# fmfi-compbio/nadavca

Hardware: AMD Instinct MI355X
Metric: reads/sec (align_signal, ~4k-sample reads) (higher is better)
Workload: dtype f64

## Files before the change

include/nadavca_hip.h:

```cpp
#ifndef NADAVCA_HIP_H
#define NADAVCA_HIP_H

#include <stddef.h>
#include <stdint.h>

#ifdef __cplusplus
extern "C" {
#endif

typedef struct nvk_ctx nvk_ctx;
typedef struct nvk_model nvk_model;

enum {
  NVK_OK = 0,
  NVK_ERR_NO_DEVICE = -1,
  NVK_ERR_INVALID = -2,
  NVK_ERR_HIP = -3,
  NVK_ERR_UNSUPPORTED = -4,
  NVK_ERR_NOMEM = -5
};

enum {
  NVK_READ_OK = 0,
  NVK_READ_NO_PATH = 1,
// ... 25 lines not shown
int nvk_ctx_synchronize(nvk_ctx *ctx);
void *nvk_ctx_stream(nvk_ctx *ctx);
int nvk_ctx_set_slots(nvk_ctx *ctx, int slots);

int nvk_timing_enable(nvk_ctx *ctx, int on);
int nvk_timing_reset(nvk_ctx *ctx);
int nvk_timing_read(nvk_ctx *ctx, int kernel_id, double *total_ms, int64_t *launches);
int nvk_last_batch_stats(nvk_ctx *ctx, int64_t *band_cells, int64_t *wave_steps,
                         int64_t *spill_bytes);
int nvk_last_retry_count(nvk_ctx *ctx, int64_t *n_reads);
enum { NVK_TIE_EXACT = 1, NVK_TIE_NEAR = 2, NVK_TIE_ULP = 4, NVK_TIE_PLATEAU = 8 };
int nvk_last_tie_count(nvk_ctx *ctx, int64_t *n_reads);
int nvk_last_tie_counts(nvk_ctx *ctx, int64_t *n_exact, int64_t *n_near, int64_t *n_ulp);
int nvk_last_tie_flags(nvk_ctx *ctx, int64_t n_reads, int32_t *out_flags);
int nvk_ctx_set_workspace_limit(nvk_ctx *ctx, int64_t bytes);

int nvk_model_create(nvk_ctx *ctx, int k, int central_position, int alphabet_size,
                     const double *mean, const double *sigma, int64_t n, nvk_model **out);
void nvk_model_destroy(nvk_model *model);
int nvk_model_info(const nvk_model *model, int *k, int *central_position, int *alphabet_size);

int nvk_expected_signal_batch(nvk_model *model, int64_t n_reads, const int32_t *reference,
                              const int64_t *ref_off, const int32_t *ctx_before,
                              const int64_t *cb_off, const int32_t *ctx_after,
                              const int64_t *ca_off, double *out);
int nvk_expected_signal_batch_dev(nvk_model *model, int64_t n_reads, int64_t total_ref,
                                  const int32_t *reference, const int64_t *ref_off,
                                  const int32_t *ctx_before, const int64_t *cb_off,
                                  const int32_t *ctx_after, const int64_t *ca_off, double *out);

// ... 104 lines not shown
```

nadavca_amd/_lib.py:

```python
import ctypes as C
import os
import threading

_HERE = os.path.dirname(os.path.abspath(__file__))
LIB_PATH = os.path.join(_HERE, 'csrc', 'libnadavca_hip.so')

NVK_OK = 0
NVK_ERR_NO_DEVICE = -1
NVK_ERR_INVALID = -2
NVK_ERR_HIP = -3
NVK_ERR_UNSUPPORTED = -4
NVK_ERR_NOMEM = -5

READ_OK = 0
READ_NO_PATH = 1
READ_BAD_INPUT = -1
READ_BAD_BAND = -2
READ_TOO_WIDE = -3

TIE_EXACT = 1
TIE_NEAR = 2
TIE_PLATEAU = 8
TIE_ULP = 4

# ... 12 lines not shown
    'nvk_device_count': (_int, []),
    'nvk_ctx_create': (_int, [_int, C.POINTER(_vp)]),
    'nvk_ctx_destroy': (None, [_vp]),
    'nvk_ctx_synchronize': (_int, [_vp]),
    'nvk_ctx_stream': (_vp, [_vp]),
    'nvk_ctx_set_slots': (_int, [_vp, _int]),
    'nvk_timing_enable': (_int, [_vp, _int]),
    'nvk_timing_reset': (_int, [_vp]),
    'nvk_timing_read': (_int, [_vp, _int, C.POINTER(_dbl), C.POINTER(_i64)]),
    'nvk_last_batch_stats': (_int, [_vp, C.POINTER(_i64), C.POINTER(_i64), C.POINTER(_i64)]),
    'nvk_last_retry_count': (_int, [_vp, C.POINTER(_i64)]),
    'nvk_last_tie_count': (_int, [_vp, C.POINTER(_i64)]),
    'nvk_last_tie_counts': (_int, [_vp, C.POINTER(_i64), C.POINTER(_i64), C.POINTER(_i64)]),
    'nvk_last_tie_flags': (_int, [_vp, _i64, _vp]),
    'nvk_ctx_set_workspace_limit': (_int, [_vp, _i64]),
    'nvk_model_create': (_int, [_vp, _int, _int, _int, _vp, _vp, _i64, C.POINTER(_vp)]),
    'nvk_model_destroy': (None, [_vp]),
    'nvk_model_info': (_int, [_vp, C.POINTER(_int), C.POINTER(_int), C.POINTER(_int)]),
    'nvk_expected_signal_batch': (_int, [_vp, _i64] + [_vp] * 7),
    'nvk_expected_signal_batch_dev': (_int, [_vp, _i64, _i64] + [_vp] * 7),
    'nvk_refine_alignment_batch': (_int, [_vp, _i64] + [_vp] * 10 + [_int, _int, _int, _vp, _vp]),
    'nvk_refine_alignment_submit': (_int, [_vp, _i64] + [_vp] * 10 + [_int, _int, _int, _vp, _vp, _vp, C.POINTER(_i64)]),
    'nvk_refine_alignment_wait': (_int, [_vp, _i64]),
    'nvk_refine_alignment_batch_dev': (_int, [_vp, _i64, _i64, _i64, _i64] + [_vp] * 10 + [_int, _int, _int, _vp, _vp]),
    'nvk_estimate_log_likelihoods_batch': (_int, [_vp, _i64] + [_vp] * 10 + [_int, _int, _int, _vp, _vp]),
    'nvk_estimate_log_likelihoods_batch_dev': (_int, [_vp, _i64, _i64, _i64, _i64] + [_vp] * 10 + [_int, _int, _int, _vp, _vp]),
    'nvk_consensus_accumulate_dev': (_int, [_vp, _i64, _i64, _int] + [_vp] * 6 + [_dbl, _i64, _vp, _vp]),
    'nvk_posterior_segments_dev': (_int, [_vp, _i64, _i64, _vp, _int, _int, _dbl, _vp, _vp, _vp]),
    'nvk_normalize_groups_dev': (_int, [_vp, _i64, _vp, _vp, _vp, _vp]),
    'nvk_select_hist_dev': (_int, [_vp, _vp, _i64, _int, _dbl, C.c_uint64, _int, _vp]),
# ... 93 lines not shown
        check(self._lib.nvk_last_retry_count(self.handle, C.byref(d)), 'nvk_last_retry_count')
        e = _i64()
        check(self._lib.nvk_last_tie_count(self.handle, C.byref(e)), 'nvk_last_tie_count')
        f, g, h = _i64(), _i64(), _i64()
        check(self._lib.nvk_last_tie_counts(self.handle, C.byref(f), C.byref(g), C.byref(h)), 'nvk_last_tie_counts')
        return dict(band_cells=a.value, wave_steps=b.value, spill_bytes=c.value, reads_redone_exact=d.value,
                    reads_tie_ambiguous=e.value, reads_tie_exact=f.value, reads_tie_near=g.value,
                    reads_tie_ulp=h.value)

    def last_tie_flags(self, n_reads):
        import numpy as np
        out = np.zeros(int(n_reads), dtype=np.int32)
        check(self._lib.nvk_last_tie_flags(self.handle, int(n_reads), _vp(out.ctypes.data)), 'nvk_last_tie_flags')
        return out

    def set_workspace_limit(self, nbytes):
        check(self._lib.nvk_ctx_set_workspace_limit(self.handle, int(nbytes)), 'nvk_ctx_set_workspace_limit')

    def close(self):
        if getattr(self, 'handle', None):
            self._lib.nvk_ctx_destroy(self.handle)
            self.handle = None

    def __del__(self):
        try:
            self.close()
        except Exception:
            pass


# ... 14 lines not shown
```

nadavca_amd/csrc/api.hip:

```cpp
#include <math.h>
#include <stdarg.h>
#include <stdio.h>
#include <stdlib.h>
#include <string.h>

#include <new>
#include <vector>

#include "nvk_internal.h"

static thread_local char g_err[512] = "";

void nvk_set_error(const char *fmt, ...) {
  va_list ap;
  va_start(ap, fmt);
  vsnprintf(g_err, sizeof g_err, fmt, ap);
  va_end(ap);
}

extern "C" const char *nvk_last_error(void) { return g_err; }

extern "C" int nvk_device_count(void) {
  int n = 0;
  if (hipGetDeviceCount(&n) != hipSuccess) return 0;
// ... 71 lines not shown
    nvk_set_error("no HIP device visible (this library has no CPU fallback)");
    return NVK_ERR_NO_DEVICE;
  }
  if (device < 0 || device >= n) {
    nvk_set_error("device %d out of range (0..%d)", device, n - 1);
    return NVK_ERR_INVALID;
  }
  NVK_HIP(hipSetDevice(device));
  nvk_ctx *c = new (std::nothrow) nvk_ctx();
  if (!c) {
    nvk_set_error("nvk_ctx_create: out of host memory");
    return NVK_ERR_NOMEM;
  }
  memset(c, 0, sizeof *c);
  c->device = device;
  hipDeviceProp_t prop;
  if (hipGetDeviceProperties(&prop, device) != hipSuccess) {
    delete c;
    nvk_set_error("hipGetDeviceProperties failed");
    return NVK_ERR_HIP;
  }
  c->num_cus = prop.multiProcessorCount > 0 ? prop.multiProcessorCount : 256;
  if (hipStreamCreate(&c->stream) != hipSuccess || hipStreamCreate(&c->stream2) != hipSuccess ||
      hipEventCreate(&c->ev0) != hipSuccess || hipEventCreate(&c->ev1) != hipSuccess ||
      hipEventCreateWithFlags(&c->ev_fork, hipEventDisableTiming) != hipSuccess ||
      hipEventCreateWithFlags(&c->ev_join, hipEventDisableTiming) != hipSuccess) {
    nvk_ctx_destroy(c);
    nvk_set_error("stream/event creation failed");
    return NVK_ERR_HIP;
  }
// ... 72 lines not shown

extern "C" int nvk_last_tie_count(nvk_ctx *ctx, int64_t *n_reads) {
  if (!ctx || !n_reads) return NVK_ERR_INVALID;
  *n_reads = ctx->last_ties;
  return NVK_OK;
}

extern "C" int nvk_last_tie_counts(nvk_ctx *ctx, int64_t *n_exact, int64_t *n_near, int64_t *n_ulp) {
  if (!ctx) return NVK_ERR_INVALID;
  if (n_exact) *n_exact = ctx->last_ties_exact;
  if (n_near) *n_near = ctx->last_ties_near;
  if (n_ulp) *n_ulp = ctx->last_ties_ulp;
  return NVK_OK;
}

extern "C" int nvk_last_tie_flags(nvk_ctx *ctx, int64_t n_reads, int32_t *out_flags) {
  if (!ctx || !out_flags || n_reads < 0) return NVK_ERR_INVALID;
  if (n_reads != ctx->ties_n) {
    nvk_set_error("nvk_last_tie_flags: the last refine_alignment batch had %lld reads, not %lld",
                  (long long)ctx->ties_n, (long long)n_reads);
    return NVK_ERR_INVALID;
  }
  if (n_reads == 0) return NVK_OK;
  if (ctx->ties_host) {
    memcpy(out_flags, ctx->ties_host, (size_t)n_reads * sizeof(int32_t));
    return NVK_OK;
  }
  NVK_HIP(hipSetDevice(ctx->device));
  NVK_HIP(hipMemcpyAsync(out_flags, ctx->ws[WS_TIES], (size_t)n_reads * sizeof(int32_t), hipMemcpyDeviceToHost,
                         ctx->stream));
// ... 155 lines not shown
}

struct PlanHost {
  PlanTotals tot;
  int32_t steps[1];
};

int plan_batch(nvk_model *model, const BatchArgs &a, int mode, int wobbling, PlanTotals &tot, const int **order,
               const int32_t **steps_sorted) {
  nvk_ctx *ctx = model->ctx;
  int64_t n = a.n_reads;
  int64_t rows_total = (mode == PLAN_ALIGN_TRANS) ? 2 * a.total_ref : a.total_ref + n;
  int rc;
  if ((rc = nvk_ws_reserve(ctx, WS_META, (size_t)(n + 1) * sizeof(ReadMeta) + 64))) return rc;
  if ((rc = nvk_ws_reserve(ctx, WS_ROWS, (size_t)(rows_total + 1) * sizeof(RowParam)))) return rc;
  if ((rc = nvk_ws_reserve(ctx, WS_BANDTMP, (size_t)(2 * (a.total_ref + n) + 2) * 8))) return rc;
  if ((rc = nvk_ws_reserve(ctx, WS_MISC, 256))) return rc;
  if ((rc = nvk_ws_reserve(ctx, WS_LANE_F, (size_t)(rows_total + 1) * 48))) return rc;
  if ((rc = nvk_ws_reserve(ctx, WS_LANE_R, (size_t)(rows_total + 1) * 48))) return rc;
  if ((rc = nvk_ws_reserve(ctx, WS_OFFS, (size_t)(rows_total + 1) * sizeof(int32_t)))) return rc;
  if ((rc = nvk_ws_reserve(ctx, WS_STEPS, (size_t)(n + 1) * sizeof(int32_t)))) return rc;
  if ((rc = nvk_grow(&ctx->h_plan, &ctx->h_plan_cap, sizeof(PlanHost) + (size_t)n * sizeof(int32_t), true,
                     "planner results")))
    return rc;
  PlanHost *hp = (PlanHost *)ctx->h_plan;
  PlanTotals *d_tot = (PlanTotals *)((char *)ctx->ws[WS_MISC] + 64);
  rc = launch_plan(ctx, model->dm, a, mode, wobbling, (ReadMeta *)ctx->ws[WS_META],
                   (RowParam *)ctx->ws[WS_ROWS], (unsigned long long *)ctx->ws[WS_BANDTMP], d_tot,
                   ctx->ws[WS_LANE_F], ctx->ws[WS_LANE_R], (int32_t *)ctx->ws[WS_OFFS]);
  if (rc) return rc;
  int *ord = nullptr;
  rc = launch_order(ctx, (const ReadMeta *)ctx->ws[WS_META], n, d_tot, &ord, (int32_t *)ctx->ws[WS_STEPS]);
  if (rc) return rc;
  NVK_HIP(hipMemcpyAsync(&hp->tot, d_tot, sizeof(PlanTotals), hipMemcpyDeviceToHost, ctx->stream));
  if (n) NVK_HIP(hipMemcpyAsync(hp->steps, ctx->ws[WS_STEPS], (size_t)n * sizeof(int32_t), hipMemcpyDeviceToHost,
                                ctx->stream));
  NVK_HIP(hipStreamSynchronize(ctx->stream));
  tot = hp->tot;
  *order = ord;
  *steps_sorted = hp->steps;
  ctx->last_cells = (int64_t)tot.cells;
  ctx->last_steps = (int64_t)tot.steps;
  return NVK_OK;
}

}

extern "C" int nvk_expected_signal_batch_dev(nvk_model *model, int64_t n_reads, int64_t total_ref,
                                             const int32_t *reference, const int64_t *ref_off,
                                             const int32_t *ctx_before, const int64_t *cb_off,
                                             const int32_t *ctx_after, const int64_t *ca_off,
                                             double *out) {
  int rc = check_common(model, n_reads, 0, 0);
  if (rc) return rc;
  nvk_ctx *ctx = model->ctx;
  NVK_HIP(hipSetDevice(ctx->device));
  rc = launch_expected(ctx, model->dm, n_reads, total_ref, reference, ref_off, ctx_before, cb_off,
// ... 99 lines not shown

extern "C" int nvk_estimate_log_likelihoods_batch_dev(
    nvk_model *model, int64_t n_reads, int64_t total_signal, int64_t total_ref,
    int64_t total_anchors, const double *signal, const int64_t *sig_off, const int32_t *reference,
    const int64_t *ref_off, const int32_t *ctx_before, const int64_t *cb_off,
    const int32_t *ctx_after, const int64_t *ca_off, const int32_t *anchors,
    const int64_t *anc_off, int bandwidth, int min_event_length, int model_wobbling,
    double *out_ll, int32_t *out_status) {
  BatchArgs a;
  int rc = dev_batch(model, n_reads, total_signal, total_ref, total_anchors, signal, sig_off, reference, ref_off,
                     ctx_before, cb_off, ctx_after, ca_off, anchors, anc_off, bandwidth, min_event_length,
                     out_status, a);
  if (rc || n_reads == 0) return rc;
  nvk_ctx *ctx = model->ctx;
  const int64_t n = n_reads, nrow = total_ref + n;
  if ((rc = nvk_ws_reserve(ctx, WS_META, (size_t)(n + 1) * sizeof(ReadMeta) + 64))) return rc;
  if ((rc = nvk_ws_reserve(ctx, WS_ROWS, (size_t)(total_ref + 1) * sizeof(FusedParam)))) return rc;
  if ((rc = nvk_ws_reserve(ctx, WS_ROWS2, (size_t)(total_ref + 1) * sizeof(FusedParam)))) return rc;
  if ((rc = nvk_ws_reserve(ctx, WS_BP, (size_t)(3 * nrow + 16) * sizeof(int32_t)))) return rc;
  if ((rc = nvk_ws_reserve(ctx, WS_BANDTMP, (size_t)(2 * nrow + 2) * 8))) return rc;
  if ((rc = nvk_ws_reserve(ctx, WS_MISC, 256))) return rc;
  EllPlan pl;
  pl.metas = (ReadMeta *)ctx->ws[WS_META];
  pl.fwd = (FusedParam *)ctx->ws[WS_ROWS];
  pl.rev = (FusedParam *)ctx->ws[WS_ROWS2];
  pl.bs = (int32_t *)ctx->ws[WS_BP];
  pl.be = pl.bs + nrow;
  pl.rowoff = pl.be + nrow;
  PlanTotals *d_tot = (PlanTotals *)((char *)ctx->ws[WS_MISC] + 64);
  rc = launch_plan_ell(ctx, model->dm, a, model_wobbling ? 1 : 0, pl,
// ... 13 lines not shown
```

nadavca_amd/csrc/kernels_plan.hip:

```cpp
#include <math.h>

#include "nvk_internal.h"
#include "lane3.h"

namespace {

__device__ __forceinline__ int seq_at(const int32_t *ref, int R, const int32_t *cb, int nb,
                                      const int32_t *ca, int na, int idx) {
  if (idx < 0) {
    int j = idx + nb;
    return j >= 0 ? cb[j] : 0;
  }
  if (idx < R) return ref[idx];
  int j = idx - R;
  return j < na ? ca[j] : 0;
}

__device__ __forceinline__ int64_t kmer_id(const DeviceModel &dm, const int32_t *ref, int R,
                                           const int32_t *cb, int nb, const int32_t *ca, int na,
                                           int pos) {
  int64_t id = 0;
  for (int j = pos - dm.central; j < pos - dm.central + dm.k; j++)
    id = id * dm.alphabet + seq_at(ref, R, cb, nb, ca, na, j);
  return id;
}

__device__ __forceinline__ int read_is_bad(const DeviceModel &dm, const BatchArgs &a, int rd, int tid,
                                           int nthreads) {
  const int64_t s0 = a.sig_off[rd], s1 = a.sig_off[rd + 1], r0 = a.ref_off[rd], r1 = a.ref_off[rd + 1];
  const int64_t a0 = a.anc_off[rd], a1 = a.anc_off[rd + 1];
  const int64_t b0 = a.cb_off[rd], b1 = a.cb_off[rd + 1], c0 = a.ca_off[rd], c1 = a.ca_off[rd + 1];
  const int64_t N64 = s1 - s0, R64 = r1 - r0;
  if (s0 < 0 || r0 < 0 || a0 < 0 || b0 < 0 || c0 < 0 || a1 < a0 || b1 < b0 || c1 < c0 ||
      s1 > a.total_signal || r1 > a.total_ref || a1 > a.total_anchors || b1 - b0 > 0x3fffffff ||
      c1 - c0 > 0x3fffffff)
    return 1;
  if (R64 < 1 || N64 < 1 || N64 > 0x3fffffff || R64 > 0x1fffffff) return 1;
  const int R = (int)R64, A = (int)(a1 - a0), nb = (int)(b1 - b0), na = (int)(c1 - c0);
  const int32_t *anc = a.anchors + 2 * a0;
  const int32_t *ref = a.reference + r0, *cb = a.ctx_before + b0, *ca = a.ctx_after + c0;
  int bad = 0;
  for (int j = tid; j < A && !bad; j += nthreads) {
    int si = anc[2 * j], ri = anc[2 * j + 1];
    if (ri < 0 || ri > R || si < -(1 << 30) || si > (1 << 30)) bad = 1;
  }
  const unsigned alpha = (unsigned)dm.alphabet;
  for (int j = tid; j < R && !bad; j += nthreads)
    if ((unsigned)ref[j] >= alpha) bad = 1;
  for (int j = tid; j < nb && !bad; j += nthreads)
    if ((unsigned)cb[j] >= alpha) bad = 1;
  for (int j = tid; j < na && !bad; j += nthreads)
    if ((unsigned)ca[j] >= alpha) bad = 1;
  return bad;
}

__device__ __forceinline__ int wave_scan_max(int v, int lane) {
  for (int d = 1; d < 64; d <<= 1) {
    int o = __shfl_up(v, d, 64);
    if (lane >= d) v = max(v, o);
  }
// ... 57 lines not shown
      v = 0x7fffffff;
    }
    v = min(wave_scan_min_rev(v, lane), carry);
    carry = __shfl(v, 0, 64);
    if (j <= R) tbe[j] = (unsigned long long)(unsigned int)v;
  }
  __syncthreads();

}

constexpr int PLAN_T = 256;
__global__ __launch_bounds__(PLAN_T) void plan_kernel(DeviceModel dm, BatchArgs a, int mode,
                                                  double log_p_in, int c_cap, ReadMeta *metas,
                                                  RowParam *rows, unsigned long long *bandtmp,
                                                  PlanTotals *totals, Lane3 *lane_f, Lane3 *lane_r,
                                                  int32_t *lane_offs) {
  const int rd = blockIdx.x;
  const int tid = threadIdx.x, lane = tid & 63;
  __shared__ unsigned long long sh_cells;
  __shared__ int sh_c;
  if (rd >= a.n_reads) return;
  if (tid == 0) {
    sh_cells = 0ull;
    sh_c = 1;
  }
  const int64_t s0 = a.sig_off[rd], r0 = a.ref_off[rd], a0 = a.anc_off[rd];
  const int64_t N64 = a.sig_off[rd + 1] - s0;
  const int64_t R64 = a.ref_off[rd + 1] - r0;
  const int64_t A64 = a.anc_off[rd + 1] - a0;
  const int nb = (int)(a.cb_off[rd + 1] - a.cb_off[rd]);
  const int na = (int)(a.ca_off[rd + 1] - a.ca_off[rd]);
  const int32_t *ref = a.reference + r0;
  const int32_t *cb = a.ctx_before + a.cb_off[rd];
  const int32_t *ca = a.ctx_after + a.ca_off[rd];
  const int32_t *anc = a.anchors + 2 * a0;
  const int N = (int)N64, R = (int)R64, A = (int)A64;
// ... 231 lines not shown
    m.rsv = plateau ? 1 : 0;
    if (badband) m.status = NVK_READ_BAD_BAND;
    metas[rd] = m;
    if (!badband) {
      atomicMax(&totals->max_steps, m.n_steps);
      atomicMax(&totals->max_c, c);
      atomicMax(&totals->max_cw, cw);
      if (c > c_cap) atomicAdd(&totals->n_wide, 1);
      atomicMax(&totals->max_T, T);
      atomicAdd(&totals->cells, (unsigned long long)cells);
      atomicAdd(&totals->steps, (unsigned long long)m.pad);
    }
  }
}


__device__ __forceinline__ void gauss_params(const DeviceModel &dm, int64_t id, double *mean,
                                             double *ac, double *mc) {
  *mean = dm.mean[id];
  *ac = dm.ac[id];
  *mc = dm.mc[id];
}

__global__ __launch_bounds__(64) void plan_ell_kernel(DeviceModel dm, BatchArgs a, int wobbling,
                                                      EllPlan pl, unsigned long long *bandtmp,
                                                      PlanTotals *totals) {
  const int rd = blockIdx.x;
  const int lane = threadIdx.x;
  if (rd >= a.n_reads) return;
  const int64_t s0 = a.sig_off[rd], r0 = a.ref_off[rd], a0 = a.anc_off[rd];
// ... 220 lines not shown
  int *ord = (int *)ctx->ws[WS_ORDER];
  int *cnt = ord + n_reads;
  NVK_HIP(hipMemsetAsync(cnt, 0, 2 * ORD_N * sizeof(int), ctx->stream));
  const unsigned blocks = (unsigned)((n_reads + 255) / 256);
  TimerScope ts(ctx, NVK_K_PLAN);
  hipLaunchKernelGGL(order_count_kernel, dim3(blocks), dim3(256), 0, ctx->stream, metas, (int)n_reads, tot_dev, cnt);
  hipLaunchKernelGGL(order_scan_kernel, dim3(1), dim3(64), 0, ctx->stream, cnt);
  hipLaunchKernelGGL(order_fill_kernel, dim3(blocks), dim3(256), 0, ctx->stream, metas, (int)n_reads, tot_dev, cnt, ord);
  if (steps_out)
    hipLaunchKernelGGL(gather_steps_kernel, dim3(blocks), dim3(256), 0, ctx->stream, metas, ord, (int)n_reads, steps_out);
  NVK_HIP(hipGetLastError());
  *order = ord;
  return NVK_OK;
}

int launch_plan(nvk_ctx *ctx, const DeviceModel &dm, const BatchArgs &a, int mode, int wobbling,
                ReadMeta *metas, RowParam *rows, unsigned long long *bandtmp, PlanTotals *totals,
                void *lane_f, void *lane_r, int32_t *lane_offs) {
  (void)wobbling;
  NVK_HIP(hipMemsetAsync(totals, 0, sizeof(PlanTotals), ctx->stream));
  if (a.n_reads == 0) return NVK_OK;
  {
    TimerScope ts(ctx, NVK_K_PLAN);
    const double log_p_in = log(0.01);
    hipLaunchKernelGGL(plan_kernel, dim3((unsigned)a.n_reads), dim3(PLAN_T), 0, ctx->stream, dm, a, mode,
                       log_p_in, ALIGN1_C_CAP, metas, rows, bandtmp, totals, (Lane3 *)lane_f, (Lane3 *)lane_r,
                       lane_offs);
  }
  NVK_HIP(hipGetLastError());
  return NVK_OK;
}

int launch_plan_ell(nvk_ctx *ctx, const DeviceModel &dm, const BatchArgs &a, int wobbling,
                    const EllPlan &pl, unsigned long long *bandtmp, PlanTotals *totals) {
  NVK_HIP(hipMemsetAsync(totals, 0, sizeof(PlanTotals), ctx->stream));
  if (a.n_reads == 0) return NVK_OK;
  {
    TimerScope ts(ctx, NVK_K_PLAN);
    hipLaunchKernelGGL(plan_ell_kernel, dim3((unsigned)a.n_reads), dim3(64), 0, ctx->stream, dm, a,
                       wobbling, pl, bandtmp, totals);
  }
  NVK_HIP(hipGetLastError());
// ... 17 lines not shown
```

nadavca_amd/csrc/lane3.h:

```cpp
#pragma once
#include "nvk_internal.h"
#include "dens.h"

struct __attribute__((aligned(16))) Lane3 {
  double mean, ac, mc;
  int32_t bs;
  int32_t end;
  int32_t lo;
  int32_t pA, pW;
  int32_t mg;
};
__device__ __forceinline__ int lane3_pack(int mel, int age, int adv) { return mel | (age << 4) | (adv * 4096); }
static_assert(sizeof(Lane3) == 48, "Lane3 layout");

__device__ __forceinline__ void set_density_consts(Lane3 &l, const RowParam &o) {
  l.mean = o.mean;
  dens::scale_consts(o.ac, o.mc, l.ac, l.mc);
  if (l.mc == 0.0) l.mean = dens::constant_density(l.ac);
}


__device__ __forceinline__ void lane3_rows(const RowParam *rw, int T, int N, int cw, Lane3 *fwdl, Lane3 *revl,
                                           int32_t *offs, int tid, int nthreads) {
  const int top = T - 1;
  const int ST = cw ? 64 * ALIGN3_TEAM_W : 64;
  for (int r = tid; r < T; r += nthreads) {
    const RowParam o = rw[r];
    Lane3 f, b;
    f.bs = o.bs; f.end = o.be; f.lo = o.lo;
    const int adv_f = (r >= ST) ? o.off - rw[r - ST].off : 0;
    const int adv_b = (r + ST <= top) ? rw[r + ST].off - o.off : 0;
    if (r > 0) {
      const RowParam p = rw[r - 1];
      set_density_consts(f, p);
      f.lo = max(o.lo, p.mel);
      {
        const int a = max(f.lo, p.bs + p.mel), z = min(o.be, p.be + p.mel);
        f.pA = (z >= a) ? a : 0x40000000; f.pW = (z >= a) ? z - a : 0;
      }
      f.mg = lane3_pack(p.mel, o.off - p.off + p.mel, adv_f);
    } else {
      f.mean = 1.0; f.ac = 0.0; f.mc = 0.0; f.mg = lane3_pack(0, 1, 0); f.pA = 0x40000000; f.pW = 0;
    }
    set_density_consts(b, o);
    b.bs = o.bs; b.lo = 0;
    if (r < top) {
      const RowParam q = rw[r + 1];
      b.end = min(o.hi, N - o.mel);
      {
        const int a = max(o.bs, q.bs - o.mel), z = min(b.end, q.be - o.mel);
        b.pA = (z >= a) ? a : 0x40000000; b.pW = (z >= a) ? z - a : 0;
      }
      b.mg = lane3_pack(o.mel, q.off - o.off + o.mel, adv_b);
    } else {
      b.pA = 0x40000000; b.pW = 0;
      b.end = o.hi;
      b.mg = lane3_pack(o.mel, 1 + o.mel, adv_b);
    }
    fwdl[r] = f;
    revl[r] = b;
    offs[r] = o.off;
  }
}
```

nadavca_amd/csrc/nvk_internal.h:

```cpp
#pragma once
#include <hip/hip_runtime.h>
#include <stdint.h>

#include "../../include/nadavca_hip.h"

struct __attribute__((aligned(16))) RowParam {
  double mean, ac, mc;
  int32_t bs, be;
  int32_t lo, hi;
  int32_t mel;
  int32_t off;
};
static_assert(sizeof(RowParam) == 48, "RowParam layout");

struct __attribute__((aligned(16))) FusedParam {
  double a_mean, a_ac, a_mc;
  double b_mean, b_ac, b_mc;
  int32_t wbs, wbe;
  int32_t ebs, ebe;
  int32_t has_wob;
  int32_t store_off;
  int32_t pad0, pad1;
};
static_assert(sizeof(FusedParam) == 80, "FusedParam layout");
// ... 46 lines not shown
  void *ws[WS_COUNT];
  size_t ws_bytes[WS_COUNT];
  int timing_on;
  double k_ms[NVK_K_COUNT];
  int64_t k_launches[NVK_K_COUNT];
  hipEvent_t ev0, ev1;
  int64_t last_cells, last_steps, last_spill_bytes;
  int64_t last_retries;
  int64_t last_ties;
  int64_t last_ties_exact, last_ties_near, last_ties_ulp;
  int64_t ties_n;
  const int32_t *ties_host;
  int64_t ws_limit;
  void *h_plan;
  size_t h_plan_cap;
  int spill_share;
  struct nvk_pipe_state *pipe;
};

struct nvk_model {
  nvk_ctx *ctx;
  DeviceModel dm;
  double *d_mean, *d_ac, *d_mc;
};


void nvk_set_error(const char *fmt, ...);
void nvk_pipe_release(nvk_ctx *ctx);
void nvk_pipe_set_ws_limit(nvk_ctx *ctx, int64_t bytes);

// ... 39 lines not shown
  const double *signal;
  const int64_t *sig_off;
  const int32_t *reference;
  const int64_t *ref_off;
  const int32_t *ctx_before;
  const int64_t *cb_off;
  const int32_t *ctx_after;
  const int64_t *ca_off;
  const int32_t *anchors;
  const int64_t *anc_off;
  int bandwidth, mel;
};

enum { PLAN_ALIGN_TRANS = 0, PLAN_ALIGN_PLAIN = 1, PLAN_ELL = 2 };

int launch_plan(nvk_ctx *ctx, const DeviceModel &dm, const BatchArgs &a, int mode, int wobbling,
                ReadMeta *metas, RowParam *rows, unsigned long long *bandtmp, PlanTotals *totals,
                void *lane_f, void *lane_r, int32_t *lane_offs);
int launch_order(nvk_ctx *ctx, const ReadMeta *metas, int64_t n_reads, const PlanTotals *tot_dev, int **order,
                 int32_t *steps_out);
int launch_align(nvk_ctx *ctx, const BatchArgs &a, int transitions, const ReadMeta *metas,
                 const RowParam *rows, const PlanTotals &tot, int32_t *out_events,
                 int32_t *out_status);
struct EllPlan {
  ReadMeta *metas;
  FusedParam *fwd;
  FusedParam *rev;
  int32_t *bs, *be;
  int32_t *rowoff;
};
// ... 19 lines not shown
```

Before: 634,000.

## Add single-wavefront plan kernel for short reads with fallback list for long reads

```diff
diff --git a/include/nadavca_hip.h b/include/nadavca_hip.h
--- a/include/nadavca_hip.h
+++ b/include/nadavca_hip.h
@@ -63,6 +63,8 @@
 int nvk_last_tie_counts(nvk_ctx *ctx, int64_t *n_exact, int64_t *n_near, int64_t *n_ulp);
 int nvk_last_tie_flags(nvk_ctx *ctx, int64_t n_reads, int32_t *out_flags);
 int nvk_ctx_set_workspace_limit(nvk_ctx *ctx, int64_t bytes);
+int nvk_last_plan_tables(nvk_ctx *ctx, int64_t *n_reads, int64_t *n_rows, void *metas, void *rows, void *lane_f,
+                         void *lane_r, void *offs, void *totals);
 
 int nvk_model_create(nvk_ctx *ctx, int k, int central_position, int alphabet_size,
                      const double *mean, const double *sigma, int64_t n, nvk_model **out);
diff --git a/nadavca_amd/_lib.py b/nadavca_amd/_lib.py
--- a/nadavca_amd/_lib.py
+++ b/nadavca_amd/_lib.py
@@ -50,6 +50,7 @@
     'nvk_last_tie_counts': (_int, [_vp, C.POINTER(_i64), C.POINTER(_i64), C.POINTER(_i64)]),
     'nvk_last_tie_flags': (_int, [_vp, _i64, _vp]),
     'nvk_ctx_set_workspace_limit': (_int, [_vp, _i64]),
+    'nvk_last_plan_tables': (_int, [_vp, C.POINTER(_i64), C.POINTER(_i64)] + [_vp] * 6),
     'nvk_model_create': (_int, [_vp, _int, _int, _int, _vp, _vp, _i64, C.POINTER(_vp)]),
     'nvk_model_destroy': (None, [_vp]),
     'nvk_model_info': (_int, [_vp, C.POINTER(_int), C.POINTER(_int), C.POINTER(_int)]),
@@ -173,6 +174,21 @@
         check(self._lib.nvk_last_tie_flags(self.handle, int(n_reads), _vp(out.ctypes.data)), 'nvk_last_tie_flags')
         return out
 
+    def last_plan_tables(self):
+        import numpy as np
+        n, nr = _i64(), _i64()
+        check(self._lib.nvk_last_plan_tables(self.handle, C.byref(n), C.byref(nr), None, None, None, None, None, None),
+              'nvk_last_plan_tables')
+        if n.value < 0:
+            raise NadavcaHipError('nvk_last_plan_tables: no align planner call on this context')
+        out = dict(metas=np.zeros((n.value, 72), np.uint8), rows=np.zeros((nr.value, 48), np.uint8),
+                   lane_f=np.zeros((nr.value, 48), np.uint8), lane_r=np.zeros((nr.value, 48), np.uint8),
+                   offs=np.zeros((nr.value, 4), np.uint8), totals=np.zeros(40, np.uint8))
+        p = lambda k: _vp(out[k].ctypes.data)
+        check(self._lib.nvk_last_plan_tables(self.handle, C.byref(n), C.byref(nr), p('metas'), p('rows'), p('lane_f'),
+                                             p('lane_r'), p('offs'), p('totals')), 'nvk_last_plan_tables')
+        return out
+
     def set_workspace_limit(self, nbytes):
         check(self._lib.nvk_ctx_set_workspace_limit(self.handle, int(nbytes)), 'nvk_ctx_set_workspace_limit')
 
diff --git a/nadavca_amd/csrc/api.hip b/nadavca_amd/csrc/api.hip
--- a/nadavca_amd/csrc/api.hip
+++ b/nadavca_amd/csrc/api.hip
@@ -109,6 +109,7 @@
   }
   memset(c, 0, sizeof *c);
   c->device = device;
+  c->plan_n = c->plan_rows = -1;
   hipDeviceProp_t prop;
   if (hipGetDeviceProperties(&prop, device) != hipSuccess) {
     delete c;
@@ -211,6 +212,27 @@
   return NVK_OK;
 }
 
+extern "C" int nvk_last_plan_tables(nvk_ctx *ctx, int64_t *n_reads, int64_t *n_rows, void *metas, void *rows,
+                                    void *lane_f, void *lane_r, void *offs, void *totals) {
+  if (!ctx || !n_reads || !n_rows) return NVK_ERR_INVALID;
+  *n_reads = ctx->plan_n;
+  *n_rows = ctx->plan_rows;
+  if (ctx->plan_n < 0) return NVK_OK;
+  NVK_HIP(hipSetDevice(ctx->device));
+  NVK_HIP(hipStreamSynchronize(ctx->stream));
+  const size_t nr = (size_t)ctx->plan_rows;
+  const struct {
+    void *dst;
+    int ws;
+    size_t bytes;
+  } tabs[] = {{metas, WS_META, (size_t)ctx->plan_n * sizeof(ReadMeta)}, {rows, WS_ROWS, nr * sizeof(RowParam)},
+              {lane_f, WS_LANE_F, nr * 48}, {lane_r, WS_LANE_R, nr * 48}, {offs, WS_OFFS, nr * sizeof(int32_t)}};
+  for (const auto &t : tabs)
+    if (t.dst && t.bytes) NVK_HIP(hipMemcpy(t.dst, ctx->ws[t.ws], t.bytes, hipMemcpyDeviceToHost));
+  if (totals) memcpy(totals, &ctx->plan_tot, sizeof(PlanTotals));
+  return NVK_OK;
+}
+
 extern "C" int nvk_last_tie_flags(nvk_ctx *ctx, int64_t n_reads, int32_t *out_flags) {
   if (!ctx || !out_flags || n_reads < 0) return NVK_ERR_INVALID;
   if (n_reads != ctx->ties_n) {
@@ -396,7 +418,9 @@
   int rc;
   if ((rc = nvk_ws_reserve(ctx, WS_META, (size_t)(n + 1) * sizeof(ReadMeta) + 64))) return rc;
   if ((rc = nvk_ws_reserve(ctx, WS_ROWS, (size_t)(rows_total + 1) * sizeof(RowParam)))) return rc;
-  if ((rc = nvk_ws_reserve(ctx, WS_BANDTMP, (size_t)(2 * (a.total_ref + n) + 2) * 8))) return rc;
+  if ((rc = nvk_ws_reserve(ctx, WS_BANDTMP,
+                           (size_t)plan_bandtmp_words(a.total_ref, n) * 8 + (size_t)(n + 1) * sizeof(int))))
+    return rc;
   if ((rc = nvk_ws_reserve(ctx, WS_MISC, 256))) return rc;
   if ((rc = nvk_ws_reserve(ctx, WS_LANE_F, (size_t)(rows_total + 1) * 48))) return rc;
   if ((rc = nvk_ws_reserve(ctx, WS_LANE_R, (size_t)(rows_total + 1) * 48))) return rc;
@@ -423,6 +447,9 @@
   *steps_sorted = hp->steps;
   ctx->last_cells = (int64_t)tot.cells;
   ctx->last_steps = (int64_t)tot.steps;
+  ctx->plan_n = n;
+  ctx->plan_rows = rows_total;
+  ctx->plan_tot = tot;
   return NVK_OK;
 }
 
@@ -552,6 +579,7 @@
   if (rc || n_reads == 0) return rc;
   nvk_ctx *ctx = model->ctx;
   const int64_t n = n_reads, nrow = total_ref + n;
+  ctx->plan_n = ctx->plan_rows = -1;
   if ((rc = nvk_ws_reserve(ctx, WS_META, (size_t)(n + 1) * sizeof(ReadMeta) + 64))) return rc;
   if ((rc = nvk_ws_reserve(ctx, WS_ROWS, (size_t)(total_ref + 1) * sizeof(FusedParam)))) return rc;
   if ((rc = nvk_ws_reserve(ctx, WS_ROWS2, (size_t)(total_ref + 1) * sizeof(FusedParam)))) return rc;
diff --git a/nadavca_amd/csrc/kernels_plan.hip b/nadavca_amd/csrc/kernels_plan.hip
--- a/nadavca_amd/csrc/kernels_plan.hip
+++ b/nadavca_amd/csrc/kernels_plan.hip
@@ -25,8 +25,7 @@
   return id;
 }
 
-__device__ __forceinline__ int read_is_bad(const DeviceModel &dm, const BatchArgs &a, int rd, int tid,
-                                           int nthreads) {
+__device__ __forceinline__ bool read_offsets_bad(const BatchArgs &a, int rd) {
   const int64_t s0 = a.sig_off[rd], s1 = a.sig_off[rd + 1], r0 = a.ref_off[rd], r1 = a.ref_off[rd + 1];
   const int64_t a0 = a.anc_off[rd], a1 = a.anc_off[rd + 1];
   const int64_t b0 = a.cb_off[rd], b1 = a.cb_off[rd + 1], c0 = a.ca_off[rd], c1 = a.ca_off[rd + 1];
@@ -34,16 +33,24 @@
   if (s0 < 0 || r0 < 0 || a0 < 0 || b0 < 0 || c0 < 0 || a1 < a0 || b1 < b0 || c1 < c0 ||
       s1 > a.total_signal || r1 > a.total_ref || a1 > a.total_anchors || b1 - b0 > 0x3fffffff ||
       c1 - c0 > 0x3fffffff)
-    return 1;
-  if (R64 < 1 || N64 < 1 || N64 > 0x3fffffff || R64 > 0x1fffffff) return 1;
-  const int R = (int)R64, A = (int)(a1 - a0), nb = (int)(b1 - b0), na = (int)(c1 - c0);
+    return true;
+  return R64 < 1 || N64 < 1 || N64 > 0x3fffffff || R64 > 0x1fffffff;
+}
+__device__ __forceinline__ bool anchor_bad(int si, int ri, int R) {
+  return ri < 0 || ri > R || si < -(1 << 30) || si > (1 << 30);
+}
+
+__device__ __forceinline__ int read_is_bad(const DeviceModel &dm, const BatchArgs &a, int rd, int tid,
+                                           int nthreads) {
+  if (read_offsets_bad(a, rd)) return 1;
+  const int64_t r0 = a.ref_off[rd], a0 = a.anc_off[rd], b0 = a.cb_off[rd], c0 = a.ca_off[rd];
+  const int R = (int)(a.ref_off[rd + 1] - r0), A = (int)(a.anc_off[rd + 1] - a0);
+  const int nb = (int)(a.cb_off[rd + 1] - b0), na = (int)(a.ca_off[rd + 1] - c0);
   const int32_t *anc = a.anchors + 2 * a0;
   const int32_t *ref = a.reference + r0, *cb = a.ctx_before + b0, *ca = a.ctx_after + c0;
   int bad = 0;
-  for (int j = tid; j < A && !bad; j += nthreads) {
-    int si = anc[2 * j], ri = anc[2 * j + 1];
-    if (ri < 0 || ri > R || si < -(1 << 30) || si > (1 << 30)) bad = 1;
-  }
+  for (int j = tid; j < A && !bad; j += nthreads)
+    if (anchor_bad(anc[2 * j], anc[2 * j + 1], R)) bad = 1;
   const unsigned alpha = (unsigned)dm.alphabet;
   for (int j = tid; j < R && !bad; j += nthreads)
     if ((unsigned)ref[j] >= alpha) bad = 1;
@@ -131,12 +138,12 @@
                                                   double log_p_in, int c_cap, ReadMeta *metas,
                                                   RowParam *rows, unsigned long long *bandtmp,
                                                   PlanTotals *totals, Lane3 *lane_f, Lane3 *lane_r,
-                                                  int32_t *lane_offs) {
-  const int rd = blockIdx.x;
+                                                  int32_t *lane_offs, const int *long_list) {
   const int tid = threadIdx.x, lane = tid & 63;
   __shared__ unsigned long long sh_cells;
   __shared__ int sh_c;
-  if (rd >= a.n_reads) return;
+  if ((int)blockIdx.x >= long_list[0]) return;
+  const int rd = long_list[1 + blockIdx.x];
   if (tid == 0) {
     sh_cells = 0ull;
     sh_c = 1;
@@ -398,6 +405,416 @@
   }
 }
 
+constexpr int PLANW_NS = 16;
+constexpr int PLANW_T = 64 * PLANW_NS;
+constexpr int planw_band_rows(int mode) { return mode == PLAN_ALIGN_TRANS ? PLANW_T / 2 + 1 : PLANW_T; }
+constexpr int PLANW_STG = 64 * 48;
+inline size_t planw_lds_bytes(int mode, int k) {
+  return PLANW_STG + sizeof(int) * (3 * (size_t)planw_band_rows(mode) + (size_t)k + PLANW_T);
+}
+
+template <class V>
+__device__ __forceinline__ V row_before(V cur, V prev_slot, int lane) {
+  const V up = __shfl_up(cur, 1, 64);
+  const V last = __shfl(prev_slot, 63, 64);
+  return lane == 0 ? last : up;
+}
+template <class V>
+__device__ __forceinline__ V row_after(V cur, V next_slot, int lane) {
+  const V dn = __shfl_down(cur, 1, 64);
+  const V first = __shfl(next_slot, 0, 64);
+  return lane == 63 ? first : dn;
+}
+__device__ __forceinline__ int wave_scan_sum(int v, int lane) {
+  for (int d = 1; d < 64; d <<= 1) {
+    const int o = __shfl_up(v, d, 64);
+    if (lane >= d) v += o;
+  }
+  return v;
+}
+__device__ __forceinline__ int wave_scan_max_rev(int v, int lane) {
+  for (int d = 1; d < 64; d <<= 1) {
+    const int o = __shfl_down(v, d, 64);
+    if (lane + d < 64) v = max(v, o);
+  }
+  return v;
+}
+
+__device__ __forceinline__ bool plan_wave_read(const BatchArgs &a, int rd, int mode) {
+  const int64_t R64 = a.ref_off[rd + 1] - a.ref_off[rd];
+  const int64_t T64 = (mode == PLAN_ALIGN_TRANS) ? 2 * R64 : R64 + 1;
+  return R64 >= 1 && T64 <= PLANW_T;
+}
+
+__global__ __launch_bounds__(64) void plan_wave_kernel(DeviceModel dm, BatchArgs a, int mode, double log_p_in,
+                                                       int c_cap, ReadMeta *metas, RowParam *rows,
+                                                       PlanTotals *totals, Lane3 *lane_f, Lane3 *lane_r,
+                                                       int32_t *lane_offs, int *long_list) {
+  constexpr int NS = PLANW_NS;
+  extern __shared__ int planw_sh[];
+  const int rd = blockIdx.x, lane = threadIdx.x;
+  if (rd >= a.n_reads) return;
+  if (!plan_wave_read(a, rd, mode)) {
+    if (lane == 0) long_list[1 + atomicAdd(long_list, 1)] = rd;
+    return;
+  }
+  const bool trans = (mode == PLAN_ALIGN_TRANS);
+  const int64_t s0 = a.sig_off[rd], r0 = a.ref_off[rd], a0 = a.anc_off[rd];
+  const int N = (int)(a.sig_off[rd + 1] - s0);
+  const int R = (int)(a.ref_off[rd + 1] - r0);
+  const int A = (int)(a.anc_off[rd + 1] - a0);
+  const int nb = (int)(a.cb_off[rd + 1] - a.cb_off[rd]);
+  const int na = (int)(a.ca_off[rd + 1] - a.ca_off[rd]);
+  const int32_t *ref = a.reference + r0;
+  const int32_t *cb = a.ctx_before + a.cb_off[rd];
+  const int32_t *ca = a.ctx_after + a.ca_off[rd];
+  const int32_t *anc = a.anchors + 2 * a0;
+  const int bw = a.bandwidth, mel = a.mel;
+
+  ReadMeta m;
+  m.sig_off = s0;
+  m.ref_off = r0;
+  m.N = N;
+  m.R = R;
+  m.status = NVK_READ_OK;
+  m.pad = 0;
+  m.cells = 0;
+  m.cw = 0;
+  m.rsv = 0;
+  const int T = trans ? 2 * R : R + 1;
+  m.row_off = trans ? 2 * r0 : r0 + rd;
+  m.T = T;
+  m.c = 1;
+  m.t_min = 0;
+  m.n_steps = 0;
+  const int NB = R + 1;
+  int4 *stg = (int4 *)planw_sh;
+  int2 *band = (int2 *)(planw_sh + PLANW_STG / sizeof(int));
+  unsigned long long *tagw = (unsigned long long *)band;
+  int *ext = (int *)(band + planw_band_rows(mode));
+  const unsigned alpha = (unsigned)dm.alphabet;
+  const int central = dm.central, tail = dm.k - central - 1;
+  bool bad = read_offsets_bad(a, rd);
+  if (!bad) {
+    for (int j = lane; j < NB; j += 64) tagw[j] = 0ull;
+    __syncthreads();
+#pragma unroll 4
+    for (int j = lane; j < A; j += 64) {
+      const int2 an = *(const int2 *)(anc + 2 * j);
+      if (anchor_bad(an.x, an.y, R))
+        bad = true;
+      else
+        atomicMax(&tagw[an.y], ((unsigned long long)(j + 1) << 32) | (unsigned int)(an.x + (1 << 30)));
+    }
+#pragma unroll 4
+    for (int j = lane; j < R; j += 64) {
+      const int v = ref[j];
+      if ((unsigned)v >= alpha) bad = true;
+      ext[central + j] = v;
+    }
+    for (int j = lane; j < nb; j += 64)
+      if ((unsigned)cb[j] >= alpha) bad = true;
+    for (int j = lane; j < na; j += 64)
+      if ((unsigned)ca[j] >= alpha) bad = true;
+    for (int j = lane; j < central; j += 64) {
+      const int i = nb - central + j;
+      ext[j] = i >= 0 ? cb[i] : 0;
+    }
+    for (int j = lane; j < tail; j += 64) ext[central + R + j] = j < na ? ca[j] : 0;
+  }
+  if (__any(bad)) {
+    m.status = NVK_READ_BAD_INPUT;
+    if (lane == 0) metas[rd] = m;
+    return;
+  }
+  __syncthreads();
+
+  for (int j = lane; j < NB; j += 64) {
+    const unsigned long long w = tagw[j];
+    int vbs = 0, vbe = N;
+    if (w >> 32) {
+      const long long sa = (long long)(unsigned int)w - (1 << 30);
+      const long long lo = sa - bw, hi = sa + bw;
+      vbs = (int)(lo > 0 ? lo : 0);
+      vbe = (int)(hi < N ? (hi < -1 ? -1 : hi) : N);
+    }
+    band[j] = make_int2(vbs, vbe);
+  }
+  __syncthreads();
+  {
+    int carry = 0;
+    for (int b0 = 0; b0 < NB; b0 += 64) {
+      const int j = b0 + lane;
+      int v = j < NB ? band[j].x : 0;
+      v = max(wave_scan_max(v, lane), carry);
+      carry = __shfl(v, 63, 64);
+      if (j < NB) band[j].x = v;
+    }
+    carry = N;
+    for (int b0 = ((NB - 1) / 64) * 64; b0 >= 0; b0 -= 64) {
+      const int j = b0 + lane;
+      int v = j < NB ? band[j].y : 0x7fffffff;
+      v = min(wave_scan_min_rev(v, lane), carry);
+      carry = __shfl(v, 0, 64);
+      if (j < NB) band[j].y = v;
+    }
+  }
+  __syncthreads();
+  auto BS = [&](int j) { return band[j].x; };
+  auto BE = [&](int j) { return band[j].y; };
+
+  auto bidx = [&](int r) { return trans ? (r + 1) >> 1 : r; };
+  auto rmel = [&](int r) { return (r + 1 < T) ? ((trans && (r & 1)) ? 0 : mel) : 0; };
+  auto span = [&](int r, int &lo, int &hi) {
+    lo = BS(bidx(r));
+    hi = BE(bidx(r));
+    if (r > 0) {
+      const int pm = rmel(r - 1);
+      lo = min(lo, BS(bidx(r - 1)) + pm) - max(pm - 1, 0);
+    }
+    if (r + 1 < T) {
+      const int pm = rmel(r);
+      hi = max(hi, BE(bidx(r + 1)) - pm) + max(pm - 1, 0);
+    }
+  };
+  const int idle = trans ? 2 : 1;
+  int badband = 0, cneed = 1;
+  long long cells = 0;
+  for (int r = lane; r < T; r += 64) {
+    const int bs = BS(bidx(r)), be = BE(bidx(r));
+    if (be < bs) badband = 1;
+    cells += (long long)(be - bs + 1);
+    if (r >= 64) {
+      int lo, hi, plo, phi;
+      span(r, lo, hi);
+      span(r - 64, plo, phi);
+      const int d = phi - lo + idle;
+      if (d >= 0) cneed = max(cneed, d / 64 + 1);
+    }
+  }
+  badband = __any(badband);
+  cells = wave_sum(cells);
+  const int c = wave_max(max(cneed, max(mel - 1, 1)));
+  const bool team = (c > c_cap);
+  int cw = 0;
+  if (team) {
+    constexpr int TL = 64 * ALIGN3_TEAM_W;
+    int need = 1;
+    for (int r = TL + lane; r < T; r += 64) {
+      int lo, hi, plo, phi;
+      span(r, lo, hi);
+      span(r - TL, plo, phi);
+      const int d = phi - lo + idle;
+      if (d >= 0) need = max(need, d / TL + 1);
+    }
+    cw = max(max(mel - 1, 1), wave_max(need));
+  }
+
+  int *offl = ext + planw_band_rows(mode) + dm.k;
+  const int gmin = max(mel - 1, 1);
+  const bool neg_gaps = trans && mel <= 2;
+  bool var_ok = false;
+  if (!team && T > 64 && (neg_gaps || c > gmin)) {
+    int x_[NS], S_[NS], k_[NS];
+    int carry = 0;
+#pragma unroll
+    for (int s = 0; s < NS; ++s) {
+      x_[s] = S_[s] = k_[s] = 0;
+      if (64 * s < T) {
+        const int r = 64 * s + lane;
+        int g = 0, lo = 0, hi = 0;
+        if (r < T) span(r, lo, hi);
+        if (r > 0 && r < T) {
+          g = gmin;
+          if (neg_gaps) {
+            int plo, phi;
+            span(r - 1, plo, phi);
+            g = max(1 - rmel(r - 1), max(plo - lo, phi - hi));
+          }
+          g = min(g, c);
+        }
+        S_[s] = wave_scan_sum(g, lane) + carry;
+        carry = __shfl(S_[s], 63, 64);
+        if (s >= 1 && r < T) {
+          int plo, phi;
+          span(r - 64, plo, phi);
+          k_[s] = phi - lo + 1 + idle - (S_[s] - S_[s - 1]);
+        }
+      }
+    }
+    const int NEG = -0x20000000;
+    bool changed = true;
+    int iter = 0;
+    while (changed && iter < 64) {
+      changed = false;
+      ++iter;
+      int carry = 0;
+#pragma unroll
+      for (int s = 0; s < NS; ++s) {
+        if (64 * s < T) {
+          const int r = 64 * s + lane;
+          const int cur = r < T ? x_[s] : NEG;
+          int v = cur;
+          if (s >= 1 && r < T) v = max(v, x_[s - 1] + k_[s]);
+          v = max(wave_scan_max(v, lane), carry);
+          if (r < T) {
+            changed |= (v != cur);
+            x_[s] = v;
+          }
+          carry = __shfl(v, 63, 64);
+        }
+      }
+      int carryz = NEG;
+#pragma unroll
+      for (int s = NS - 1; s >= 0; --s) {
+        if (64 * s < T) {
+          const int r = 64 * s + lane;
+          const int cur = r < T ? x_[s] : 0;
+          const int U = r < T ? c * r - S_[s] : 0;
+          int z = r < T ? cur - U : NEG;
+          z = max(wave_scan_max_rev(z, lane), carryz);
+          if (r < T) {
+            const int nx = z + U;
+            changed |= (nx != cur);
+            x_[s] = nx;
+          }
+          carryz = __shfl(z, 0, 64);
+        }
+      }
+      changed = __any(changed);
+    }
+    var_ok = !changed;
+    if (var_ok) {
+      const int x0 = __shfl(x_[0], 0, 64);
+#pragma unroll
+      for (int s = 0; s < NS; ++s)
+        if (64 * s + lane < T) offl[64 * s + lane] = x_[s] - x0 + S_[s];
+    }
+  }
+  if (!var_ok) {
+    const int cu = team ? cw : c;
+    for (int r = lane; r < T; r += 64) offl[r] = cu * r;
+  }
+  __syncthreads();
+
+  RowParam *rp = rows + m.row_off;
+  const bool lanes = lane_f && !badband;
+  Lane3 *fl = lanes ? lane_f + m.row_off : nullptr, *rl = lanes ? lane_r + m.row_off : nullptr;
+  int32_t *ol = lanes ? lane_offs + m.row_off : nullptr;
+  const int top = T - 1;
+  const int ST = cw ? 64 * ALIGN3_TEAM_W : 64;
+  int plateau = 0;
+  auto gather = [&](int r, double &gm, double &ga, double &gc) {
+    int64_t id = 0;
+    if (r + 1 < T) {
+      const int pos = trans ? (r + 1) >> 1 : r;
+      for (int t = 0; t < dm.k; ++t) id = id * dm.alphabet + ext[pos + t];
+    }
+    gm = dm.mean[id];
+    ga = dm.ac[id];
+    gc = dm.mc[id];
+  };
+  double nm, na_, nc;
+  gather(lane, nm, na_, nc);
+  double gm_prev = 0.0, pm_prev = 0.0, pa_prev = 0.0, pc_prev = 0.0;
+  for (int r = lane; r - lane < T; r += 64) {
+    const double cm = nm, ca_ = na_, cc = nc;
+    if (r + 64 - lane < T) gather(r + 64, nm, na_, nc);
+    const bool live = r < T;
+    const bool step = r + 1 < T, emits = step && !(trans && (r & 1));
+    const double gm = step ? cm : 0.0, ga = emits ? ca_ : 0.0, gc = emits ? cc : 0.0;
+    const double gm_before = row_before(gm, gm_prev, lane);
+    gm_prev = gm;
+    double pmean = gm, pac = ga, pmc = gc;
+    if (step) {
+      if (trans && (r & 1)) {
+        pac = (gm_before == gm) ? -INFINITY : log_p_in;
+        pmean = 0.0;
+        plateau |= (gm_before == gm) ? 1 : 0;
+      } else if (!trans && r >= 1) {
+        plateau |= (gm_before == gm) ? 1 : 0;
+      }
+    }
+    const double qm = row_before(pmean, pm_prev, lane), qa = row_before(pac, pa_prev, lane),
+                 qc = row_before(pmc, pc_prev, lane);
+    pm_prev = pmean;
+    pa_prev = pac;
+    pc_prev = pmc;
+    const int nlive = min(64, T - (r - lane));
+    auto put = [&](void *dst) {
+      __syncthreads();
+      int4 *d = (int4 *)dst + 3 * (r - lane);
+      for (int q = lane; q < 3 * nlive; q += 64) d[q] = stg[q];
+      __syncthreads();
+    };
+    RowParam o;
+    if (live) {
+      o.mean = pmean;
+      o.ac = pac;
+      o.mc = pmc;
+      o.bs = BS(bidx(r));
+      o.be = BE(bidx(r));
+      span(r, o.lo, o.hi);
+      o.mel = rmel(r);
+      o.off = offl[r];
+      ((RowParam *)stg)[lane] = o;
+    }
+    put(rp);
+    if (lanes) {
+      Lane3 f, b;
+      if (live) {
+        RowParam p = o, q = o;
+        if (r > 0) {
+          p.mean = qm;
+          p.ac = qa;
+          p.mc = qc;
+          p.bs = BS(bidx(r - 1));
+          p.be = BE(bidx(r - 1));
+          p.mel = rmel(r - 1);
+          p.off = offl[r - 1];
+        }
+        if (r < top) {
+          q.bs = BS(bidx(r + 1));
+          q.be = BE(bidx(r + 1));
+          q.off = offl[r + 1];
+        }
+        const int adv_f = (r >= ST) ? o.off - offl[r - ST] : 0;
+        const int adv_b = (r + ST <= top) ? offl[r + ST] - o.off : 0;
+        lane3_row(o, p, r > 0, q, r < top, N, adv_f, adv_b, f, b);
+        ((Lane3 *)stg)[lane] = f;
+        ol[r] = o.off;
+      }
+      put(fl);
+      if (live) ((Lane3 *)stg)[lane] = b;
+      put(rl);
+    }
+  }
+  plateau = __any(plateau);
+
+  if (lane == 0) {
+    const int t_min = BS(0);
+    const int hi_top = BE(bidx(top));
+    m.c = c;
+    m.cw = cw;
+    m.t_min = t_min;
+    m.n_steps = hi_top + c * top - t_min + 1;
+    m.pad = (hi_top + offl[top] - t_min + 1 + 31) & ~31;
+    m.cells = cells;
+    m.rsv = plateau ? 1 : 0;
+    if (badband) m.status = NVK_READ_BAD_BAND;
+    metas[rd] = m;
+    if (!badband) {
+      atomicMax(&totals->max_steps, m.n_steps);
+      atomicMax(&totals->max_c, c);
+      atomicMax(&totals->max_cw, cw);
+      if (c > c_cap) atomicAdd(&totals->n_wide, 1);
+      atomicMax(&totals->max_T, T);
+      atomicAdd(&totals->cells, (unsigned long long)cells);
+      atomicAdd(&totals->steps, (unsigned long long)m.pad);
+    }
+  }
+}
+
 
 __device__ __forceinline__ void gauss_params(const DeviceModel &dm, int64_t id, double *mean,
                                              double *ac, double *mc) {
@@ -648,18 +1065,26 @@
   return NVK_OK;
 }
 
+int64_t plan_bandtmp_words(int64_t total_ref, int64_t n_reads) { return 2 * (total_ref + n_reads) + 2; }
+
 int launch_plan(nvk_ctx *ctx, const DeviceModel &dm, const BatchArgs &a, int mode, int wobbling,
                 ReadMeta *metas, RowParam *rows, unsigned long long *bandtmp, PlanTotals *totals,
                 void *lane_f, void *lane_r, int32_t *lane_offs) {
   (void)wobbling;
   NVK_HIP(hipMemsetAsync(totals, 0, sizeof(PlanTotals), ctx->stream));
   if (a.n_reads == 0) return NVK_OK;
+  int *long_list = (int *)(bandtmp + plan_bandtmp_words(a.total_ref, a.n_reads));
+  NVK_HIP(hipMemsetAsync(long_list, 0, sizeof(int), ctx->stream));
   {
     TimerScope ts(ctx, NVK_K_PLAN);
     const double log_p_in = log(0.01);
-    hipLaunchKernelGGL(plan_kernel, dim3((unsigned)a.n_reads), dim3(PLAN_T), 0, ctx->stream, dm, a, mode,
-                       log_p_in, ALIGN1_C_CAP, metas, rows, bandtmp, totals, (Lane3 *)lane_f, (Lane3 *)lane_r,
-                       lane_offs);
+    const size_t lds = planw_lds_bytes(mode, dm.k);
+    hipLaunchKernelGGL(plan_wave_kernel, dim3((unsigned)a.n_reads), dim3(64), lds, ctx->stream, dm, a, mode,
+                       log_p_in, ALIGN1_C_CAP, metas, rows, totals, (Lane3 *)lane_f, (Lane3 *)lane_r, lane_offs,
+                       long_list);
+    hipLaunchKernelGGL(plan_kernel, dim3((unsigned)a.n_reads), dim3(PLAN_T), 0, ctx->stream, dm, a, mode, log_p_in,
+                       ALIGN1_C_CAP, metas, rows, bandtmp, totals, (Lane3 *)lane_f, (Lane3 *)lane_r, lane_offs,
+                       (const int *)long_list);
   }
   NVK_HIP(hipGetLastError());
   return NVK_OK;
diff --git a/nadavca_amd/csrc/lane3.h b/nadavca_amd/csrc/lane3.h
--- a/nadavca_amd/csrc/lane3.h
+++ b/nadavca_amd/csrc/lane3.h
@@ -20,43 +20,49 @@
 }
 
 
+__device__ __forceinline__ void lane3_row(const RowParam &o, const RowParam &p, bool has_p, const RowParam &q,
+                                          bool has_q, int N, int adv_f, int adv_b, Lane3 &f, Lane3 &b) {
+  f.bs = o.bs; f.end = o.be; f.lo = o.lo;
+  if (has_p) {
+    set_density_consts(f, p);
+    f.lo = max(o.lo, p.mel);
+    {
+      const int a = max(f.lo, p.bs + p.mel), z = min(o.be, p.be + p.mel);
+      f.pA = (z >= a) ? a : 0x40000000; f.pW = (z >= a) ? z - a : 0;
+    }
+    f.mg = lane3_pack(p.mel, o.off - p.off + p.mel, adv_f);
+  } else {
+    f.mean = 1.0; f.ac = 0.0; f.mc = 0.0; f.mg = lane3_pack(0, 1, 0); f.pA = 0x40000000; f.pW = 0;
+  }
+  set_density_consts(b, o);
+  b.bs = o.bs; b.lo = 0;
+  if (has_q) {
+    b.end = min(o.hi, N - o.mel);
+    {
+      const int a = max(o.bs, q.bs - o.mel), z = min(b.end, q.be - o.mel);
+      b.pA = (z >= a) ? a : 0x40000000; b.pW = (z >= a) ? z - a : 0;
+    }
+    b.mg = lane3_pack(o.mel, q.off - o.off + o.mel, adv_b);
+  } else {
+    b.pA = 0x40000000; b.pW = 0;
+    b.end = o.hi;
+    b.mg = lane3_pack(o.mel, 1 + o.mel, adv_b);
+  }
+}
+
 __device__ __forceinline__ void lane3_rows(const RowParam *rw, int T, int N, int cw, Lane3 *fwdl, Lane3 *revl,
                                            int32_t *offs, int tid, int nthreads) {
   const int top = T - 1;
   const int ST = cw ? 64 * ALIGN3_TEAM_W : 64;
   for (int r = tid; r < T; r += nthreads) {
     const RowParam o = rw[r];
-    Lane3 f, b;
-    f.bs = o.bs; f.end = o.be; f.lo = o.lo;
     const int adv_f = (r >= ST) ? o.off - rw[r - ST].off : 0;
     const int adv_b = (r + ST <= top) ? rw[r + ST].off - o.off : 0;
-    if (r > 0) {
-      const RowParam p = rw[r - 1];
-      set_density_consts(f, p);
-      f.lo = max(o.lo, p.mel);
-      {
-        const int a = max(f.lo, p.bs + p.mel), z = min(o.be, p.be + p.mel);
-        f.pA = (z >= a) ? a : 0x40000000; f.pW = (z >= a) ? z - a : 0;
-      }
-      f.mg = lane3_pack(p.mel, o.off - p.off + p.mel, adv_f);
-    } else {
-      f.mean = 1.0; f.ac = 0.0; f.mc = 0.0; f.mg = lane3_pack(0, 1, 0); f.pA = 0x40000000; f.pW = 0;
-    }
-    set_density_consts(b, o);
-    b.bs = o.bs; b.lo = 0;
-    if (r < top) {
-      const RowParam q = rw[r + 1];
-      b.end = min(o.hi, N - o.mel);
-      {
-        const int a = max(o.bs, q.bs - o.mel), z = min(b.end, q.be - o.mel);
-        b.pA = (z >= a) ? a : 0x40000000; b.pW = (z >= a) ? z - a : 0;
-      }
-      b.mg = lane3_pack(o.mel, q.off - o.off + o.mel, adv_b);
-    } else {
-      b.pA = 0x40000000; b.pW = 0;
-      b.end = o.hi;
-      b.mg = lane3_pack(o.mel, 1 + o.mel, adv_b);
-    }
+    RowParam p, q;
+    if (r > 0) p = rw[r - 1];
+    if (r < top) q = rw[r + 1];
+    Lane3 f, b;
+    lane3_row(o, p, r > 0, q, r < top, N, adv_f, adv_b, f, b);
     fwdl[r] = f;
     revl[r] = b;
     offs[r] = o.off;
diff --git a/nadavca_amd/csrc/nvk_internal.h b/nadavca_amd/csrc/nvk_internal.h
--- a/nadavca_amd/csrc/nvk_internal.h
+++ b/nadavca_amd/csrc/nvk_internal.h
@@ -84,6 +84,8 @@
   int64_t ws_limit;
   void *h_plan;
   size_t h_plan_cap;
+  int64_t plan_n, plan_rows;
+  PlanTotals plan_tot;
   int spill_share;
   struct nvk_pipe_state *pipe;
 };
@@ -153,6 +155,7 @@
 
 enum { PLAN_ALIGN_TRANS = 0, PLAN_ALIGN_PLAIN = 1, PLAN_ELL = 2 };
 
+int64_t plan_bandtmp_words(int64_t total_ref, int64_t n_reads);
 int launch_plan(nvk_ctx *ctx, const DeviceModel &dm, const BatchArgs &a, int mode, int wobbling,
                 ReadMeta *metas, RowParam *rows, unsigned long long *bandtmp, PlanTotals *totals,
                 void *lane_f, void *lane_r, int32_t *lane_offs);
```

Result: faster. 641,200 (median of 6 runs) (+1.1%).
